# yanx27/PointASNL

Hardware: AMD Instinct MI355X
Metric: point-clouds/sec fwd (Bx1024 pts, ModelNet40 cls) (higher is better)
Workload: dtype f32; 1 GPU; configs[1]: ModelNet40 pointasnl_cls, 1024 pts, batch=64/GPU, seeded random weights; global_batch=64, parallelism=batch-shard x1, RCCL all-gather of logits, pipeline=prefetch, hip_graph=True, prefix_forked_at=start, prefix_levels=2, settle_replays=40, hip_hw_queues=4

## Files before the change

### include/pasnl.h

```cpp
#ifndef PASNL_H_
#define PASNL_H_

#include <stddef.h>
#include <stdint.h>

#ifdef __cplusplus
extern "C" {
#endif

#define PASNL_VERSION 100

enum {
  PASNL_OK = 0,
  PASNL_EINVAL = -1,
  PASNL_ENULL = -2,
  PASNL_EWORKSPACE = -3,
  PASNL_ELAUNCH = -4,
  PASNL_EUNSUPPORTED = -5
};

typedef void* pasnl_stream_t;

int pasnl_version(void);
const char* pasnl_strerror(int code);
// ... 92 lines not shown

int pasnl_sa_project(int b, int n, int c, int c1, const float* xyz, const float* feature, const float* w0, const float* b0,
                     float* proj, pasnl_stream_t stream);
int pasnl_sa_cell_pre(int b, int n, int c, int m, int k, int c1, int c2, const float* xyz, const float* feature,
                      const float* proj, const int* idx, const float* new_xyz, const float* w0, const float* w1, const float* b1,
                      const float* ww, const float* bw, float* out, float* skip_max, pasnl_stream_t stream);
int pasnl_sa_cell_pre_centre0(int b, int n, int c, int m, int k, int c1, int c2, const float* xyz, const float* feature,
                              const float* proj, const int* idx, const float* w0, const float* w1, const float* b1,
                              const float* ww, const float* bw, float* out, float* skip_max, float* new_xyz, float* new_feature,
                              pasnl_stream_t stream);

int pasnl_sa_cell_packed(int b, int n, int c, int npoint, int nsample, int c1, int c2, const float* xyz, const float* feature,
                         const int* idx, const float* new_xyz, const float* w0, const float* b0, const float* w1, const float* b1,
                         const float* ww, const float* bw, const float* w0_features_packed, const float* w1_packed, float* out,
                         float* skip_max, float* new_xyz_out, float* new_feature_out, pasnl_stream_t stream);

int pasnl_max_pool_rows(int b, int n, int c, const float* x, float* out, pasnl_stream_t stream);

int pasnl_max_pool_rows_strided(int b, int n, int c, const float* x, float* out, long out_stride, pasnl_stream_t stream);

size_t pasnl_mlp3_packed_weights_bytes(int k, int n);
int pasnl_mlp3_pack_weights(int k, int n, const float* w, float* packed, pasnl_stream_t stream);
size_t pasnl_mlp3_max_pool_workspace_bytes(int b, int n, int c3);
int pasnl_mlp3_max_pool(int b, int n, int k0, int c1, int c2, int c3, const float* x, const float* w0, const float* b0,
                        const float* w1, const float* b1, const float* w2, const float* b2, float* out, long out_stride,
                        void* workspace, size_t workspace_bytes, pasnl_stream_t stream);

int pasnl_cls_tail_group_all(int b, int n, int w, int cb, int c, const float* after, const float* skip_max, const float* att,
                             const float* ws_packed, const float* bs, const float* wb_packed, const float* bb,
                             const float* wagg_packed, const float* bagg, const float* new_xyz, int c1, int c2, int c3,
                             const float* w0, const float* b0, const float* w1, const float* b1, const float* w2, const float* b2,
                             float* out, float* pooled, long pooled_stride, void* workspace, size_t workspace_bytes,
                             pasnl_stream_t stream);

size_t pasnl_bf16x3_weights_bytes(int kdim, int n);
int pasnl_bf16x3_split_weights(int kdim, int n, const float* w, void* wsplit, pasnl_stream_t stream);
int pasnl_dense_bf16x3(int rows, int kdim, int n, int lda, const float* x, const void* wsplit, const float* bias, int relu,
                       float* out, pasnl_stream_t stream);


size_t pasnl_dense_rows_workspace_bytes(int rows, int kdim, int n);
int pasnl_dense_rows(int rows, int kdim, int n, const float* x, const float* w, const float* bias, int relu, float* out,
                     void* workspace, size_t workspace_bytes, pasnl_stream_t stream);

size_t pasnl_dense_splitk_workspace_bytes(int rows, int kdim, int n);
int pasnl_dense_splitk(int rows, int kdim, int n, int lda, const float* x, const float* w, const float* bias, int relu,
                       float* out, void* workspace, size_t workspace_bytes, pasnl_stream_t stream);

int pasnl_narrow_project2(long rows0, int kdim0, int n0, const float* x0, const float* w0, const float* bias0, float* out0,
                          long rows1, int kdim1, int n1, const float* x1, const float* w1, const float* bias1, float* out1,
                          pasnl_stream_t stream);

int pasnl_cls_nl_cell_input(int b, int p, int n, int c, int cz, int cb, const float* feature, const float* new_point,
                            const float* wkv, const float* bkv, const float* wq, const float* bq, float* out,
                            pasnl_stream_t stream);

size_t pasnl_cls_nl_cell_input_grad_workspace_bytes(int b, int p, int n, int c, int cz, int cb);
int pasnl_cls_nl_cell_input_grad(int b, int p, int n, int c, int cz, int cb, const float* feature, const float* new_point,
                                 const float* wkv, const float* bkv, const float* wq, const float* bq, const float* grad_out,
                                 float* grad_feature, float* grad_new_point, float* grad_wkv, float* grad_bkv, float* grad_wq,
                                 float* grad_bq, void* workspace, size_t workspace_bytes, pasnl_stream_t stream);

size_t pasnl_cls_nl_attention_grad_workspace_bytes(int b, int p, int n, int cb);
int pasnl_cls_nl_attention_grad(int b, int p, int n, int cb, const float* q, const float* kv, const float* out,
                                const float* grad_out, float* grad_q, float* grad_kv, void* workspace, size_t workspace_bytes,
                                pasnl_stream_t stream);
// ... 315 lines not shown
```

### pointasnl_amd/_hip.py

```python
import ctypes
import os

import torch

_HERE = os.path.dirname(os.path.abspath(__file__))
LIB_PATH = os.path.join(_HERE, "csrc", "libpasnl_hip.so")

SYMBOLS = [
    "pasnl_version", "pasnl_strerror", "pasnl_device_count",
    "pasnl_farthest_point_sample", "pasnl_farthest_point_sample_gather", "pasnl_gather_point", "pasnl_gather_point_grad", "pasnl_prob_sample",
    "pasnl_query_ball_point", "pasnl_sa_group", "pasnl_group_point", "pasnl_group_point_grad", "pasnl_select_top_k", "pasnl_knn_batch", "pasnl_knn_workspace_bytes", "pasnl_knn_batch_ws", "pasnl_knn_batch_ws_bg", "pasnl_knn_tree_workspace_bytes", "pasnl_knn_batch_tree", "pasnl_knn_batch_ref_workspace_bytes", "pasnl_knn_batch_ref", "pasnl_knn_distance_pick",
    "pasnl_three_nn", "pasnl_three_interpolate", "pasnl_three_interpolate_grad", "pasnl_three_weights", "pasnl_fp_interpolate_cat",
    "pasnl_nl_attention", "pasnl_nl_attention_workspace_bytes", "pasnl_nl_attention_ws", "pasnl_as_attention", "pasnl_as_reweight", "pasnl_sa_local_cell", "pasnl_sa_cell", "pasnl_sa_cell_centre0", "pasnl_sa_cell_packed", "pasnl_sa_project", "pasnl_sa_cell_pre", "pasnl_sa_cell_pre_centre0", "pasnl_sa_tail", "pasnl_sa_tail_cat", "pasnl_sa_tail_res", "pasnl_sa_tail_packed_weights_bytes", "pasnl_sa_tail_pack_weights", "pasnl_sa_tail_packed", "pasnl_decode_cell", "pasnl_decode_cell_tiled", "pasnl_decode_cell_tiled_v4", "pasnl_max_pool_rows", "pasnl_max_pool_rows_strided", "pasnl_mlp3_max_pool_workspace_bytes", "pasnl_mlp3_max_pool", "pasnl_mlp3_packed_weights_bytes", "pasnl_mlp3_pack_weights", "pasnl_dense_rows_workspace_bytes", "pasnl_dense_rows", "pasnl_dense_splitk_workspace_bytes", "pasnl_dense_splitk", "pasnl_bf16x3_weights_bytes", "pasnl_bf16x3_split_weights", "pasnl_dense_bf16x3", "pasnl_narrow_project2", "pasnl_take_neighbor0", "pasnl_as_gather", "pasnl_as_attention_qkv", "pasnl_as_attention_proj", "pasnl_as_cell_narrow", "pasnl_as_cell_wide", "pasnl_as_cell_wide_ld", "pasnl_as_reweight_x", "pasnl_grid_subsample_workspace_bytes", "pasnl_grid_subsample", "pasnl_knn_crop_workspace_bytes", "pasnl_knn_crop",
    "pasnl_scan_pick", "pasnl_knn_crop_indirect", "pasnl_crop_order_permute", "pasnl_scan_possibility_update", "pasnl_scan_scratch_init", "pasnl_scan_vote", "pasnl_scan_reproject_workspace_bytes", "pasnl_scan_reproject", "pasnl_scan_labels",
    "pasnl_scan_pick_given", "pasnl_scan_train_labels", "pasnl_scan_augment",
    "pasnl_scan_eval_confusion", "pasnl_scene_eval_vote", "pasnl_scene_eval_vote_confusion",
    "pasnl_scan_radius_workspace_bytes", "pasnl_scan_radius_members", "pasnl_scene_radius_members", "pasnl_scan_radius_gather", "pasnl_scene_radius_gather",
    "pasnl_scene_pick", "pasnl_knn_crop_scene", "pasnl_scene_pick_crop", "pasnl_scene_order_gather", "pasnl_scene_potential_update", "pasnl_scene_vote", "pasnl_scene_labels", "pasnl_confusion_matrix",
    "pasnl_window_noise", "pasnl_window_bounds", "pasnl_window_hist_bytes", "pasnl_window_count", "pasnl_window_fill", "pasnl_window_gather", "pasnl_window_vote", "pasnl_window_pool_labels",
    "pasnl_kwindow_hist_bytes", "pasnl_kwindow_count", "pasnl_kwindow_fill", "pasnl_kwindow_gather",
    "pasnl_modelnet_fps_cap", "pasnl_modelnet_fps", "pasnl_modelnet_normalize", "pasnl_modelnet_batch", "pasnl_modelnet_augment", "pasnl_modelnet_noise", "pasnl_cls_vote", "pasnl_cls_tally",
    "pasnl_cls_tail_group_all", "pasnl_cls_nl_cell_input", "pasnl_cls_nl_cell_input_grad_workspace_bytes", "pasnl_cls_nl_cell_input_grad", "pasnl_cls_nl_attention_grad_workspace_bytes", "pasnl_cls_nl_attention_grad",
    "pasnl_cls_as_attention_grad", "pasnl_cls_as_attention_qkv_grad", "pasnl_cls_as_reweight_grad", "pasnl_cls_as_reweight_x_grad", "pasnl_cls_as_gather_grad_workspace_bytes", "pasnl_cls_as_gather_grad",
    "pasnl_cls_sa_local_cell_grad_workspace_bytes", "pasnl_cls_sa_local_cell_grad", "pasnl_cls_sa_group_grad_workspace_bytes", "pasnl_cls_sa_group_grad",
    "pasnl_block_key_capacity", "pasnl_block_crop_stats", "pasnl_block_grid_count", "pasnl_block_fill", "pasnl_block_gather", "pasnl_block_normalize", "pasnl_block_score_workspace_bytes", "pasnl_block_score", "pasnl_block_train_batch", "pasnl_block_train_score",
    "pasnl_kblock_crop_stats", "pasnl_kblock_grid_count", "pasnl_kblock_fill", "pasnl_kblock_gather", "pasnl_kblock_rotate",
    "pasnl_grad_workspace_bytes", "pasnl_gather_point_grad_det", "pasnl_group_point_grad_det", "pasnl_three_interpolate_grad_det",
]


class PasnlError(RuntimeError):
    pass


class PasnlUnsupported(PasnlError):
    """PASNL_EUNSUPPORTED: a valid request outside what the fused kernel covers (include/pasnl.h documents the limits).
    The cells catch it and take their op-by-op path (still HIP kernels + vendor GEMMs, never a CPU path)."""


_lib = None


def lib():
    global _lib
    if _lib is None:
        if not os.path.exists(LIB_PATH):
            raise PasnlError(
                f"{LIB_PATH} is missing: build it with `python -c 'import __graft_entry__ as g; g.build()'` "
                "(or `make -C pointasnl_amd/csrc`).  pointasnl_amd has no CPU or eager fallback.")
        _lib = ctypes.CDLL(LIB_PATH)
        _lib.pasnl_strerror.restype = ctypes.c_char_p
        _lib.pasnl_grad_workspace_bytes.restype = ctypes.c_size_t
        _lib.pasnl_knn_workspace_bytes.restype = ctypes.c_size_t
        _lib.pasnl_knn_tree_workspace_bytes.restype = ctypes.c_size_t
        _lib.pasnl_knn_batch_ref_workspace_bytes.restype = ctypes.c_size_t
# ... 126 lines not shown
```

### pointasnl_amd/csrc/mlp_pool.hip

```cpp
#include "common.hpp"
#include "sa_tail.hpp"

namespace pasnl {

typedef float mp_f32x16 __attribute__((ext_vector_type(16)));

__device__ __forceinline__ int mp_kappa(int t, int h) { return (t & 3) + 8 * (t >> 2) + 4 * h; }

template <int WOUT, int NB, int RB>
__device__ __forceinline__ void mp_mm(const float* xrow, int rbstride, int NBT, const float* __restrict__ Wp, const int (&loff)[NB],
                                      mp_f32x16 (&acc)[RB][NB]) {
  constexpr int BT = 8;
  float xb[2][RB][BT];
  float4 wa[2][NB][2];
  auto load = [&](int set, int bt) {
    const float* wrow = Wp + (size_t)bt * (16 * WOUT);
#pragma unroll
    for (int i = 0; i < NB; ++i) {
      wa[set][i][0] = *reinterpret_cast<const float4*>(wrow + loff[i]);
      wa[set][i][1] = *reinterpret_cast<const float4*>(wrow + loff[i] + 4);
    }
#pragma unroll
    for (int u = 0; u < BT; ++u)
#pragma unroll
      for (int rb = 0; rb < RB; ++rb)
        xb[set][rb][u] = xrow[rb * rbstride + 2 * (bt * BT + u)];
  };
  load(0, 0);
  for (int bt = 0; bt < NBT; bt += 2) {
#pragma unroll
    for (int half = 0; half < 2; ++half) {
      const int b0 = bt + half;
      if (b0 < NBT) {
        load(half ^ 1, min(b0 + 1, NBT - 1));
        __builtin_amdgcn_sched_barrier(0);
#pragma unroll
        for (int u = 0; u < BT; ++u) {
          float wv[NB];
#pragma unroll
          for (int i = 0; i < NB; ++i) {
            const float4 q = wa[half][i][u >> 2];
            wv[i] = (u & 3) == 0 ? q.x : ((u & 3) == 1 ? q.y : ((u & 3) == 2 ? q.z : q.w));
          }
#pragma unroll
          for (int rb = 0; rb < RB; ++rb)
#pragma unroll
            for (int i = 0; i < NB; ++i)
              acc[rb][i] = __builtin_amdgcn_mfma_f32_32x32x2f32(xb[half][rb][u], wv[i], acc[rb][i], 0, 0, 0);
        }
        __builtin_amdgcn_sched_barrier(0);
      }
    }
  }
}

template <int WOUT, int RB>
__device__ __forceinline__ void mp_layer(const float* in, int pin, int K, const float* __restrict__ W, const float* __restrict__ bias,
                                         float* out, int pout, int wave, int ql, int h) {
  constexpr int NW = 8, BLOCKS = WOUT / 32, NB = BLOCKS >= NW ? BLOCKS / NW : 1;
  if constexpr (BLOCKS * RB == NW && RB > 1) {
    const int rb = wave / BLOCKS;
    mp_layer<WOUT, 1>(in + rb * 32 * pin, pin, K, W, bias, out + rb * 32 * pout, pout, wave % BLOCKS, ql, h);
    return;
  }
  if (wave >= BLOCKS) return;
  int loff[NB];
  mp_f32x16 acc[RB][NB];
#pragma unroll
  for (int i = 0; i < NB; ++i) {
    loff[i] = (h * WOUT + (wave + NW * i) * 32 + ql) * 8;
#pragma unroll
    for (int rb = 0; rb < RB; ++rb)
#pragma unroll
      for (int r = 0; r < 16; ++r) acc[rb][i][r] = 0.f;
  }
  mp_mm<WOUT, NB, RB>(in + ql * pin + h, 32 * pin, (K + 15) >> 4, W, loff, acc);
#pragma unroll
  for (int i = 0; i < NB; ++i) {
    const int ch = (wave + NW * i) * 32 + ql;
    const float bb = bias[ch];
#pragma unroll
    for (int rb = 0; rb < RB; ++rb)
#pragma unroll
      for (int r = 0; r < 16; ++r) out[(rb * 32 + mp_kappa(r, h)) * pout + ch] = fmaxf(acc[rb][i][r] + bb, 0.f);
  }
}

template <int C1, int C2, int C3, int RB>
__device__ __forceinline__ void mlp3_tile(float* A, int pa, float* Bf, int k0, const float* __restrict__ w0, const float* __restrict__ b0,
                                          const float* __restrict__ w1, const float* __restrict__ b1, const float* __restrict__ w2,
                                          const float* __restrict__ b2, float* __restrict__ po, int wave, int ql, int h) {
  constexpr int NW = 8, PB = C1 + 1;
  mp_layer<C1, RB>(A, pa, k0, w0, b0, Bf, PB, wave, ql, h);
  __syncthreads();
  mp_layer<C2, RB>(Bf, PB, C1, w1, b1, A, pa, wave, ql, h);
  __syncthreads();
  constexpr int NB = C3 / 32 / NW;
  int loff[NB];
  mp_f32x16 acc[RB][NB];
#pragma unroll
  for (int i = 0; i < NB; ++i) {
    loff[i] = (h * C3 + (wave + NW * i) * 32 + ql) * 8;
#pragma unroll
    for (int rb = 0; rb < RB; ++rb)
#pragma unroll
      for (int r = 0; r < 16; ++r) acc[rb][i][r] = 0.f;
  }
  mp_mm<C3, NB, RB>(A + ql * pa + h, 32 * pa, C2 >> 4, w2, loff, acc);
#pragma unroll
  for (int i = 0; i < NB; ++i) {
    float mx = acc[0][i][0];
#pragma unroll
    for (int rb = 0; rb < RB; ++rb)
#pragma unroll
      for (int r = 0; r < 16; ++r) mx = fmaxf(mx, acc[rb][i][r]);
    mx = fmaxf(mx, __shfl_xor(mx, 32));
    const int ch = (wave + NW * i) * 32 + ql;
// ... 94 lines not shown
    for (int i = 0; i < 16; ++i) v[i] = fmaxf(acc[i], 0.f);
#pragma unroll
    for (int i = 0; i < 16; ++i) acc[i] = bb[cbase + kappa(i, h)];
    acc = tail_product(TailW<true>{Wb, C, TG_CB, h, cbase + l32}, nt_, l32, acc);
#pragma unroll
    for (int i = 0; i < 16; ++i) v[i] += fmaxf(acc[i], 0.f);
#pragma unroll
    for (int i = 0; i < 16; ++i) {
      float* cell = vt + (cbase + kappa(i, h)) * 33 + l32;
      *cell = *cell + v[i];
    }
  }
  __syncthreads();
  {
    f32x16 o;
#pragma unroll
    for (int i = 0; i < 16; ++i) o[i] = bagg[cbase + kappa(i, h)];
    o = tail_product(TailW<true>{Wagg, C, C, h, cbase + l32}, vt, l32, o);
    float* xr = A + (rb * 32 + l32) * pa + 4 + cbase;
#pragma unroll
    for (int i = 0; i < 16; ++i) xr[kappa(i, h)] = fmaxf(o[i], 0.f);
  }
  __syncthreads();
#pragma unroll
  for (int i = 0; i < RPW; ++i) {
    const int r = wave * RPW + i, row = tile * TG_TR + r;
    if (row < n) {
      float* o = out + (cloud0 + row) * C;
      o[lane] = A[r * pa + 4 + lane];
      o[64 + lane] = A[r * pa + 4 + 64 + lane];
    }
  }
  mlp3_tile<TG_C, TG_C2, TG_C3, 2>(A, pa, Bf, TG_K0, w0, b0, w1, b1, w2, b2, partial + ((size_t)cloud * gridDim.x + tile) * TG_C3, wave, l32, h);
}

__global__ __launch_bounds__(256) void mlp3_pack_kernel(int K, int N, const float* __restrict__ W, float* __restrict__ P) {
  const long total = (long)((K + 15) >> 4) * 2 * N * 2;
  for (long e = (long)blockIdx.x * 256 + threadIdx.x; e < total; e += (long)gridDim.x * 256) {
    const int half = (int)(e & 1);
    const long lane = e >> 1;
    const int n = (int)(lane % N);
    const long bh = lane / N;
    const int h = (int)(bh & 1), bt = (int)(bh >> 1);
    float v[4];
#pragma unroll
    for (int j = 0; j < 4; ++j) {
      const int k = 16 * bt + 2 * (4 * half + j) + h;
      v[j] = k < K ? W[(size_t)k * N + n] : 0.f;
    }
    reinterpret_cast<float4*>(P)[e] = make_float4(v[0], v[1], v[2], v[3]);
  }
}

template <int C1, int C2, int C3, int RB>
static int mlp3_launch(int b, int n, int k0, const float* x, const float* w0, const float* b0, const float* w1, const float* b1,
                       const float* w2, const float* b2, float* partial, hipStream_t st) {
  const int k0p = (k0 + 15) & ~15;
  const int pa = (k0p > C2 ? k0p : C2) | 1;
  const size_t lds = ((size_t)32 * RB * pa + (size_t)32 * RB * (C1 + 1)) * sizeof(float);
  if (lds > LDS_MAX_BYTES) return PASNL_EUNSUPPORTED;
  if (launch(mlp3_pool_kernel<C1, C2, C3, RB>, dim3((n + 32 * RB - 1) / (32 * RB), b), dim3(512), lds, st, n, k0, x, w0, b0, w1, b1,
             w2, b2, partial) != PASNL_OK)
    return PASNL_ELAUNCH;
  return pasnl_launch_status();
}

// ... 36 lines not shown
  float* partial = static_cast<float*>(workspace);
  int rc;
  int tr;
  if (c1 == 128 && c2 == 256 && c3 == 512) { tr = 64; rc = mlp3_launch<128, 256, 512, 2>(b, n, k0, x, w0, b0, w1, b1, w2, b2, partial, st); }
  else if (c1 == 256 && c2 == 512 && c3 == 1024) { tr = 32; rc = mlp3_launch<256, 512, 1024, 1>(b, n, k0, x, w0, b0, w1, b1, w2, b2, partial, st); }
  else return PASNL_EUNSUPPORTED;
  if (rc != PASNL_OK) return rc;
  return pasnl_max_pool_rows_strided(b, (n + tr - 1) / tr, c3, partial, out, out_stride, stream);
}

extern "C" int pasnl_cls_tail_group_all(int b, int n, int w, int cb, int c, const float* after, const float* skip_max, const float* att,
                                        const float* ws_packed, const float* bs, const float* wb_packed, const float* bb,
                                        const float* wagg_packed, const float* bagg, const float* new_xyz, int c1, int c2, int c3,
                                        const float* w0, const float* b0, const float* w1, const float* b1, const float* w2,
                                        const float* b2, float* out, float* pooled, long pooled_stride, void* workspace,
                                        size_t workspace_bytes, pasnl_stream_t stream) {
  PASNL_REQUIRE(b >= 0 && n > 0 && w > 0 && cb > 0 && c > 0 && c1 > 0 && c2 > 0 && c3 > 0 && pooled_stride >= c3, PASNL_EINVAL);
  if (b == 0) return PASNL_OK;
  PASNL_REQUIRE(after && skip_max && att && ws_packed && bs && wb_packed && bb && wagg_packed && bagg && new_xyz, PASNL_ENULL);
  PASNL_REQUIRE(w0 && b0 && w1 && b1 && w2 && b2 && out && pooled && workspace, PASNL_ENULL);
  PASNL_REQUIRE(workspace_bytes >= pasnl_mlp3_max_pool_workspace_bytes(b, n, c3), PASNL_EWORKSPACE);
  PASNL_REQUIRE(w == TG_W && cb == TG_CB && c == TG_C && c1 == TG_C && c2 == TG_C2 && c3 == TG_C3, PASNL_EUNSUPPORTED);
  PASNL_REQUIRE(b <= 65535, PASNL_EUNSUPPORTED);
  PASNL_REQUIRE((reinterpret_cast<uintptr_t>(ws_packed) | reinterpret_cast<uintptr_t>(wb_packed) | reinterpret_cast<uintptr_t>(wagg_packed) |
                 reinterpret_cast<uintptr_t>(w0) | reinterpret_cast<uintptr_t>(w1) | reinterpret_cast<uintptr_t>(w2)) % 16 == 0,
                PASNL_EUNSUPPORTED);
  const int tiles = (n + TG_TR - 1) / TG_TR;
  if (launch(tail_group_all_kernel, dim3(tiles, b), dim3(512), TG_LDS_BYTES, pasnl_hip_stream(stream), n, after, skip_max, att, ws_packed,
             bs, wb_packed, bb, wagg_packed, bagg, new_xyz, w0, b0, w1, b1, w2, b2, out, static_cast<float*>(workspace)) != PASNL_OK)
    return PASNL_ELAUNCH;
  if (pasnl_launch_status() != PASNL_OK) return PASNL_ELAUNCH;
  return pasnl_max_pool_rows_strided(b, tiles, c3, static_cast<const float*>(workspace), pooled, pooled_stride, stream);
}
```

### pointasnl_amd/models/pointasnl_cls.py

```python
import torch

from pointasnl_amd.utils import tf_util, pointasnl_util
from pointasnl_amd.utils.pointnet_util import pointnet_sa_module
from pointasnl_amd.utils.pointasnl_util import PointASNLSetAbstraction, get_repulsion_loss, sa_search, Forked


def first_layer(num_point=None):
    return dict(npoint=512, nsample=32)


def get_model(point_cloud, is_training=False, use_normal=False, bn_decay=None, weight_decay=None, num_class=40,
              adaptive_sample=False, search=None, before_head=None, fork_at="head", lazy_fork=None):
    if lazy_fork is None:
        lazy_fork = not adaptive_sample
    batch_size = point_cloud.shape[0]
    end_points = {}
    if use_normal:
        l0_xyz = point_cloud[:, :, 0:3].contiguous()
        l0_points = point_cloud[:, :, 3:6].contiguous()
    else:
        l0_xyz = point_cloud
        l0_points = point_cloud
    end_points['l0_xyz'] = l0_xyz
    as_neighbor = [12, 12] if adaptive_sample else [0, 0]

    net = torch.empty((batch_size, 1024 + 512), dtype=torch.float32, device=point_cloud.device)
    fuse3_1 = not adaptive_sample or pointasnl_util.SA_TAIL_GROUP_ALL == "always"
    nl_input_space = not adaptive_sample or pointasnl_util.NL_INPUT_SPACE == "always"

    search2 = []
    if isinstance(search, dict):
        search2.append(search[2])
        search = search[1]
    l1_xyz, l1_points = PointASNLSetAbstraction(l0_xyz, l0_points, npoint=512, nsample=32, mlp=[64, 64, 128],
                                                is_training=is_training, bn_decay=bn_decay, weight_decay=weight_decay,
                                                scope='layer1', as_neighbor=as_neighbor[0], search=search, xyz_concat=True,
                                                nl_input_space=nl_input_space,
                                                group_all=dict(mlp=[128, 256, 512], scope='layer3_1', pooled_out=net[:, 1024:]) if fuse3_1 else None,
                                                after_sampling=None if search2 else lambda xyz1: search2.append(
                                                    Forked(lambda: sa_search(xyz1, None, 128, 64), lazy=lazy_fork)))
    end_points['l1_xyz'] = l1_xyz
    l2_xyz, l2_points = PointASNLSetAbstraction(l1_xyz, l1_points, npoint=128, nsample=64, mlp=[128, 128, 256],
                                                is_training=is_training, bn_decay=bn_decay, weight_decay=weight_decay,
                                                scope='layer2', as_neighbor=as_neighbor[1], search=search2[0], xyz_concat=True,
                                                after_cell=before_head if fork_at == "cell2" else None,
                                                before_after_conv=before_head if fork_at == "conv2" else None)
    end_points['l2_xyz'] = l1_xyz
    if before_head is not None and fork_at == "head":
        before_head()
    if getattr(l1_points, "group_all_pooled", None) is None:
        _, l3_points_res, _ = pointnet_sa_module(l1_xyz, l1_points, npoint=None, radius=None, nsample=None,
                                                 mlp=[128, 256, 512], mlp2=None, group_all=True, is_training=is_training,
                                                 bn_decay=bn_decay, scope='layer3_1', pooled_out=net[:, 1024:])
    _, l3_points, _ = pointnet_sa_module(l2_xyz, l2_points, npoint=None, radius=None, nsample=None,
                                         mlp=[256, 512, 1024], mlp2=None, group_all=True, is_training=is_training,
                                         bn_decay=bn_decay, scope='layer3_2', pooled_out=net[:, :1024])

    net = tf_util.fully_connected(net, 512, bn=True, is_training=is_training, scope='fc1', bn_decay=bn_decay)
    net = tf_util.dropout(net, keep_prob=0.4, is_training=is_training, scope='dp1')
    net = tf_util.fully_connected(net, 256, bn=True, is_training=is_training, scope='fc2', bn_decay=bn_decay)
    net = tf_util.dropout(net, keep_prob=0.4, is_training=is_training, scope='dp2')
    net = tf_util.fully_connected(net, num_class, activation_fn=None, scope='fc3')
    end_points['l1_points'] = l1_points
    end_points['l2_points'] = l2_points
    end_points['l2_xyz_true'] = l2_xyz
    return net, end_points


def get_loss(pred, label, end_points, uniform_weight=0, weights_decay=1e-4):
    regularization_loss = tf_util.regularization_loss(weights_decay)
    loss = torch.nn.functional.cross_entropy(pred, label.long(), reduction='none')
    classify_loss = loss.mean()
    if uniform_weight > 0:
        uniform_loss = get_repulsion_loss(end_points['l1_xyz'], nsample=20, radius=0.07)
    else:
        uniform_loss = classify_loss
    return classify_loss + uniform_weight * uniform_loss + regularization_loss
```

### pointasnl_amd/utils/pointasnl_util.py

```python

import ctypes

import torch

from pointasnl_amd import _hip
from pointasnl_amd import tf_sampling, tf_grouping, nearest_neighbors
from pointasnl_amd.tf_interpolate import three_nn, three_interpolate, three_weights, fp_interpolate_cat
from pointasnl_amd.utils import tf_util, pointnet_util

NL_KEY_PARTS = True
NL_VARIANT = 0


KNN_TIE_ORDER = "reference"


def knn_query(k, support_pts, query_pts, out=None, max_workgroups=None):
    return nearest_neighbors.knn_batch(support_pts, query_pts, k, omp=True, dtype=torch.int32, tie_order=KNN_TIE_ORDER, out=out,
                                       max_workgroups=max_workgroups)


def _gather_rows(points, idx):
    return tf_grouping.group_point(points, idx.unsqueeze(-1)).squeeze(2)

# ... 65 lines not shown
                    _hip.ptr(grad_new_xyz), _hip.ptr(ws), ctypes.c_size_t(nbytes))
        return grad_xyz, grad_feature, None, grad_new_xyz


def sa_group(xyz, feature, idx, new_xyz):
    if _needs_grad(xyz, feature, new_xyz):
        b, n, c = feature.shape
        _, p, k = idx.shape
        if _grad_entry_supported("pasnl_cls_sa_group_grad", b, n, c, p, k):
            return _SAGroup.apply(xyz, feature, idx, new_xyz)
        grouped_xyz = tf_grouping.group_point(xyz, idx)
        new_point = torch.cat([grouped_xyz - new_xyz.unsqueeze(2), grouped_xyz, tf_grouping.group_point(feature, idx)], dim=-1)
        return new_point, new_point.amax(dim=2)
    return _sa_group_forward(xyz, feature, idx, new_xyz)


def _sa_group_forward(xyz, feature, idx, new_xyz):
    b, n, c = feature.shape
    _, p, k = idx.shape
    xyz, feature, idx, new_xyz = xyz.contiguous(), feature.contiguous(), idx.contiguous(), new_xyz.contiguous()
    new_point = torch.empty((b, p, k, 6 + c), dtype=torch.float32, device=xyz.device)
    skip = torch.empty((b, p, 6 + c), dtype=torch.float32, device=xyz.device)
    _hip.launch("pasnl_sa_group", "sa_group", b, n, c, p, k, _hip.ptr(xyz), _hip.ptr(feature), _hip.ptr(idx),
                _hip.ptr(new_xyz), _hip.ptr(new_point), _hip.ptr(skip))
    return new_point, skip


SELF_KNN_RATIO = 2
SA_TAIL_MIN_ROWS = 2048
FP_HEAD_FUSED = True
SA_CELL_PACKED = True
SA_TAIL_PACKED = True
SA_TAIL_GROUP_ALL = True
SA_TAIL_FUSED = True
SA_CELL_GATHER = True
SA_CELL_SINGLE = True
SA_CELL_WIDE = True
LOCAL_CELL_FUSED = True


def _local_cell_supported(w, mlp, nsample):
    if not LOCAL_CELL_FUSED or nsample % 32:
        return False
    wide = (256, 512) if SA_CELL_WIDE else ()
    if len(mlp) == 3:
        return mlp[0] == mlp[1] and mlp[0] in (16, 32, 64, 128) + wide
    return len(mlp) == 2 and mlp[0] in (32, 64, 128) + wide


class _SALocalCell(torch.autograd.Function):

    @staticmethod
    def forward(ctx, new_point, w0, b0, w1, b1, ww, bw):
        args = tuple(t.contiguous() for t in (new_point, w0, b0, w1, b1, ww, bw))
        ctx.save_for_backward(*args)
        return _sa_local_cell_forward(*args)

    @staticmethod
    @torch.autograd.function.once_differentiable
    def backward(ctx, grad_out):
        x, w0, b0, w1, b1, ww, bw = ctx.saved_tensors
        b, p, k, w = x.shape
        c1, c2 = w0.shape[1], w1.shape[1]
        grad_out = grad_out.contiguous()
        grads = [torch.empty_like(t) if need else None for t, need in zip((x, w0, b0, w1, b1, ww, bw), ctx.needs_input_grad)]
        nbytes = int(_hip.lib().pasnl_cls_sa_local_cell_grad_workspace_bytes(b * p, w, c1, c2)) if any(ctx.needs_input_grad[1:]) else 0
# ... 807 lines not shown
def sa_search_split(xyz, npoint, nsample, knn_all, slot=0):
    fp = Forked(lambda: tf_sampling.farthest_point_sample_gather(npoint, xyz), slot=slot)

    def join():
        fps_idx, new_xyz = fp.get()
        k_all = _resolved(knn_all)
        idx = _gather_index_rows(k_all, fps_idx)
        if k_all.shape[2] != nsample:
            idx = idx[:, :, :nsample].contiguous()
        return new_xyz, None, idx
    return Deferred(join)


def _tail_packed(st, w):
    key = "@tailpk:%x" % w.data_ptr()
    if key not in st._folded:
        wc = w.contiguous()
        pk = torch.empty(int(_hip.lib().pasnl_sa_tail_packed_weights_bytes(wc.shape[0], wc.shape[1])) // 4, dtype=torch.float32,
                         device=w.device)
        _hip.launch("pasnl_sa_tail_pack_weights", "sa_tail_pack", int(wc.shape[0]), int(wc.shape[1]), _hip.ptr(wc), _hip.ptr(pk))
        st._folded[key] = (pk, w)
    return st._folded[key][0]


def PointASNLSetAbstraction(xyz, feature, npoint, nsample, mlp, is_training, bn_decay, weight_decay, scope, bn=True,
                            use_knn=True, radius=None, as_neighbor=8, NL=True, search=None, after_sampling=None,
                            xyz_concat=False, after_cell=None, before_after_conv=None, residual=None, group_all=None,
                            nl_input_space=True):
    ga_weights = None
    if (group_all is not None and SA_TAIL_GROUP_ALL and SA_TAIL_FUSED and SA_TAIL_PACKED and NL and residual is None and not is_training
            and mlp[-1] == 128 and tuple(group_all['mlp']) == (128, 256, 512)):
        with tf_util.variable_scope(group_all['scope']):
            ga_weights = pointnet_util.group_all_weights(group_all['mlp'], 3 + mlp[-1], 1, bn)
    with tf_util.variable_scope(scope):
        batch_size, num_points, num_channel = feature.shape
        new_xyz, _, idx = _resolved(search) if search is not None else sa_search(xyz, feature, npoint, nsample, use_knn, radius)
        new_feature = feature
        nl_channel = mlp[-1]
        st_path = tf_util.store().path("")
        diff = not is_training and torch.is_grad_enabled() and (
            xyz.requires_grad or feature.requires_grad
            or any(v.requires_grad for name, v in tf_util.store().vars.items() if name.startswith(st_path)))

        fused = _local_cell_supported(6 + num_channel, mlp, nsample)
        centre0 = False
        if num_points != npoint and as_neighbor == 0:
            xyz, feature, idx = xyz.contiguous(), feature.contiguous(), idx.contiguous()

            def take0():
                nx = torch.empty((batch_size, npoint, 3), dtype=torch.float32, device=xyz.device)
                nf = torch.empty((batch_size, npoint, 3 + num_channel), dtype=torch.float32, device=xyz.device)
                _hip.launch("pasnl_take_neighbor0", "take_neighbor0", batch_size, num_points, num_channel, npoint, nsample,
                            _hip.ptr(xyz), _hip.ptr(feature), _hip.ptr(idx), _hip.ptr(nx), _hip.ptr(nf))
                return nx, nf
            centre0 = (not diff and CENTRE0 and fused and SA_CELL_GATHER and npoint <= num_points
                       and (num_channel <= 128 or (SA_CELL_WIDE and mlp[0] in (256, 512) and nsample == 32)))
            if diff:
                idx0 = idx[:, :, 0].contiguous()
                new_xyz = _gather_rows(xyz, idx0)
                new_feature = torch.cat([new_xyz, _gather_rows(feature, idx0)], dim=-1)
            elif not centre0:
                new_xyz, new_feature = take0()
        elif num_points != npoint and AS_FUSED and as_neighbor <= 16:
            tf_util._require_inference(is_training)
            new_xyz, new_feature = adaptive_sampling_fused(xyz, feature, idx, as_neighbor, scope, bn, weight_decay)
        elif num_points != npoint:
# ... 60 lines not shown
                                   is_training=is_training, scope='after_conv', bn_decay=bn_decay, weight_decay=weight_decay)
            st = tf_util.store()
            w_in = skip_spatial.shape[-1]
            with tf_util.variable_scope('skip'):
                ws, bs = st.layer(w_in, c_out, bn, weight_decay)
            if NL:
                with tf_util.variable_scope(scope), tf_util.variable_scope('conv_back_project'):
                    wb, bb = st.layer(cb, c_out, bn, weight_decay)
            with tf_util.variable_scope('aggregation'):
                wagg, bagg = st.layer(c_out, c_out, bn, weight_decay)
            rows = batch_size * npoint
            after, skip_spatial = after.contiguous(), skip_spatial.contiguous()
            att = att.contiguous() if NL else None
            out = torch.empty((batch_size, npoint, c_out), dtype=torch.float32, device=xyz.device)
            args = (rows, int(w_in), int(cb if NL else 0), int(c_out), _hip.ptr(after), _hip.ptr(skip_spatial),
                    _hip.ptr(att), _hip.ptr(ws), _hip.ptr(bs), _hip.ptr(wb if NL else None),
                    _hip.ptr(bb if NL else None), _hip.ptr(wagg), _hip.ptr(bagg), _hip.ptr(out))
            try:
                if SA_TAIL_PACKED:
                    pk = [_tail_packed(st, m) if m is not None else None for m in (ws, wb if NL else None, wagg)]
                    cat = None
                    if ga_weights is not None and (int(w_in), int(cb)) == (9, 32) and new_xyz.shape[1] == npoint:
                        new_xyz = new_xyz.contiguous()
                        gmlp = group_all['mlp']
                        pooled = pointnet_util.group_all_pooled(group_all.get('pooled_out'), batch_size, gmlp[-1], xyz.device)
                        wsb = pointnet_util.group_all_workspace(batch_size, npoint, gmlp[-1], xyz.device)
                        _hip.launch("pasnl_cls_tail_group_all", "sa_tail_group_all", batch_size, npoint, int(w_in), int(cb), int(c_out),
                                    *args[4:7], _hip.ptr(pk[0]), args[8], _hip.ptr(pk[1]), args[10], _hip.ptr(pk[2]), args[12],
                                    _hip.ptr(new_xyz), gmlp[0], gmlp[1], gmlp[2], *[_hip.ptr(t) for t in ga_weights], args[13],
                                    _hip.ptr(pooled), ctypes.c_long(pooled.stride(0) if batch_size > 1 else gmlp[-1]),
                                    _hip.ptr(wsb), ctypes.c_size_t(wsb.numel()))
                        out.group_all_pooled = pooled
                        return new_xyz, out
                    if xyz_concat and XYZ_CONCAT:
                        new_xyz = new_xyz.contiguous()
                        cat = torch.empty((batch_size, npoint, 4 + c_out), dtype=torch.float32, device=xyz.device)
                    res_c = residual.contiguous() if residual is not None else None
                    _hip.launch("pasnl_sa_tail_packed", "sa_tail", *args[:7], _hip.ptr(pk[0]), args[8], _hip.ptr(pk[1]), args[10],
                                _hip.ptr(pk[2]), args[12], _hip.ptr(res_c), _hip.ptr(new_xyz if cat is not None else None),
                                _hip.ptr(cat), args[13])
                    residual = None
                    if cat is not None:
                        out.xyz_concat = (new_xyz, cat)
                elif residual is not None:
                    residual = residual.contiguous()
                    _hip.launch("pasnl_sa_tail_res", "sa_tail", *args[:-1], _hip.ptr(residual), args[-1])
                    residual = None
                elif xyz_concat and XYZ_CONCAT:
                    new_xyz = new_xyz.contiguous()
                    cat = torch.empty((batch_size, npoint, 4 + c_out), dtype=torch.float32, device=xyz.device)
                    _hip.launch("pasnl_sa_tail_cat", "sa_tail", *args, _hip.ptr(new_xyz), _hip.ptr(cat))
                    out.xyz_concat = (new_xyz, cat)
                else:
                    _hip.launch("pasnl_sa_tail", "sa_tail", *args)
            except _hip.PasnlUnsupported:
                tail = after.reshape(rows, c_out) + torch.relu_(torch.addmm(bs, skip_spatial.reshape(rows, w_in), ws))
                if NL:
                    tail = tail + torch.relu_(torch.addmm(bb, att.reshape(rows, cb), wb))
                out = torch.relu_(torch.addmm(bagg, tail, wagg)).reshape(batch_size, npoint, c_out)
            return new_xyz, (out if residual is None else out + residual)

        if NL:
            new_nonlocal_point = PointNonLocalCell(feature, new_feature.unsqueeze(1),
                                                   [max(32, num_channel // 2), nl_channel], is_training, bn_decay,
                                                   weight_decay, scope, bn, input_space=nl_input_space)

# ... 117 lines not shown
```

### pointasnl_amd/utils/pointnet_util.py

```python
import ctypes

import torch

from pointasnl_amd.tf_sampling import farthest_point_sample, farthest_point_sample_gather, gather_point
from pointasnl_amd.tf_grouping import query_ball_point, group_point, knn_point
from pointasnl_amd.tf_interpolate import three_nn, three_interpolate, three_weights, fp_interpolate_cat
from pointasnl_amd.utils import tf_util
from pointasnl_amd import _hip


def sample_and_group(npoint, radius, nsample, xyz, points, knn=False, use_xyz=True):
    _, new_xyz = farthest_point_sample_gather(npoint, xyz)
    if knn:
        _, idx = knn_point(nsample, xyz, new_xyz)
    else:
        idx, pts_cnt = query_ball_point(radius, nsample, xyz, new_xyz)
    grouped_xyz = group_point(xyz, idx)
    grouped_xyz = grouped_xyz - new_xyz.unsqueeze(2)
    if points is not None:
        grouped_points = group_point(points, idx)
        new_points = torch.cat([grouped_xyz, grouped_points], dim=-1) if use_xyz else grouped_points
    else:
        new_points = grouped_xyz
    return new_xyz, new_points, idx, grouped_xyz
# ... 32 lines not shown
                if key not in st._folded:
                    st._folded[key] = (torch.cat([w.new_zeros((pad, w.shape[1])), w], dim=0).contiguous(), bb)
                w, bb = st._folded[key]
            key = st.path("") + "@mlp3:%x" % w.data_ptr()
            if key not in st._folded:
                wc = w.contiguous()
                pk = torch.empty(int(_hip.lib().pasnl_mlp3_packed_weights_bytes(wc.shape[0], wc.shape[1])) // 4, dtype=torch.float32,
                                 device=w.device)
                _hip.launch("pasnl_mlp3_pack_weights", "mlp3_pack", int(wc.shape[0]), int(wc.shape[1]), _hip.ptr(wc), _hip.ptr(pk))
                st._folded[key] = (pk, w)
            w = st._folded[key][0]
        ws += [w, bb]
        cin = c
    return ws


def group_all_pooled(pooled_out, b, c3, device):
    if pooled_out is None:
        return torch.empty((b, c3), dtype=torch.float32, device=device)
    if tuple(pooled_out.shape) != (b, c3) or pooled_out.stride(1) != 1 or pooled_out.dtype != torch.float32:
        raise ValueError("group_all_mlp_max: pooled_out must be a (B, C) float32 view with unit column stride")
    return pooled_out


def group_all_workspace(b, n, c3, device):
    nbytes = int(_hip.lib().pasnl_mlp3_max_pool_workspace_bytes(b, n, c3))
    key = (device.index, torch.cuda.current_stream().cuda_stream, c3)
    bufs = _GROUP_ALL_WS.setdefault(key, [])
    if not bufs or bufs[-1].numel() < nbytes:
        bufs.append(torch.empty(max(nbytes, 256), dtype=torch.uint8, device=device))
    return bufs[-1]


def group_all_mlp_max(new_points, mlp, bn, pooled_out=None):
    b, one, n, kp = new_points.shape
    if one != 1 or len(mlp) != 3:
        raise _hip.PasnlUnsupported("group_all_mlp_max: one group per cloud, three convolutions")
    pad = getattr(new_points, "input_pad", 0)
    ws = group_all_weights(mlp, kp - pad, pad, bn)
    x = new_points.reshape(b, n, kp)
    if not x.is_contiguous():
        x = x.contiguous()
    c3 = mlp[-1]
    out2d = group_all_pooled(pooled_out, b, c3, x.device)
    wsb = group_all_workspace(b, n, c3, x.device)
    _hip.launch("pasnl_mlp3_max_pool", "mlp3_max_pool", b, n, kp, mlp[0], mlp[1], mlp[2], _hip.ptr(x), *[_hip.ptr(t) for t in ws],
                _hip.ptr(out2d), ctypes.c_long(out2d.stride(0) if b > 1 else c3), _hip.ptr(wsb), ctypes.c_size_t(wsb.numel()))
    return out2d.unflatten(0, (b, 1)).unsqueeze(2)


def sample_and_group_all(xyz, points, use_xyz=True):
    batch_size, nsample = xyz.shape[0], xyz.shape[1]
    key = (batch_size, nsample, str(xyz.device))
    if key not in _GROUP_ALL_CONST:
        new_xyz = torch.zeros((batch_size, 1, 3), dtype=torch.float32, device=xyz.device)
        idx = torch.arange(nsample, dtype=torch.int32, device=xyz.device).reshape(1, 1, nsample).repeat(batch_size, 1, 1)
        _GROUP_ALL_CONST[key] = (new_xyz, idx)
    new_xyz, idx = _GROUP_ALL_CONST[key]
    grouped_xyz = xyz.reshape(batch_size, 1, nsample, 3)
    pre = getattr(points, "xyz_concat", None) if (points is not None and use_xyz) else None
    if pre is not None and pre[0] is xyz:
        new_points = pre[1].unsqueeze(1)
        new_points.input_pad = 1
    elif points is not None:
        new_points = torch.cat([xyz, points], dim=2) if use_xyz else points
        new_points = new_points.unsqueeze(1)
# ... 55 lines not shown
```

### pointasnl_amd/utils/tf_util.py

```python
import contextlib
import hashlib
import math

import numpy as np
import torch

from pointasnl_amd import _hip

BN_EPS = 1e-3
FUSE_RELU_EPILOGUE = True
WEIGHTS_TRANSPOSED_MIN_K = 2048


class VariableStore:

    def __init__(self, seed=0, device="cuda", randomize_bn=False):
        self.seed = int(seed)
        self.device = device
        self.randomize_bn = randomize_bn
        self.vars = {}
        self.decays = {}
        self._folded = {}
        self._scope = []

    @contextlib.contextmanager
    def scope(self, name):
        self._scope.append(name)
        try:
            yield
        finally:
            self._scope.pop()

    def path(self, name):
        return "/".join(self._scope + [name])

    def _rng(self, full):
        h = hashlib.sha256(f"{self.seed}:{full}".encode()).digest()
        return np.random.Generator(np.random.PCG64(int.from_bytes(h[:8], "little")))

    def load(self, variables, strict=True):
        for name in getattr(variables, "files", None) or variables.keys():
            leaf = name.split(":")[0].split("/")[-1]
            if leaf not in ("weights", "biases", "beta", "gamma", "moving_mean", "moving_variance"):
                continue
            a = np.asarray(variables[name], dtype=np.float32)
            if leaf == "weights" and a.ndim > 2:
                a = a.reshape(-1, a.shape[-1])
            self.vars[name.split(":")[0]] = torch.tensor(a, dtype=torch.float32, device=self.device)
        self.strict = bool(strict)
        self._folded.clear()
        return self

    def assign(self, full_name, value):
        self.vars[full_name] = torch.as_tensor(value, dtype=torch.float32).to(self.device).contiguous()
        self._folded.clear()

    strict = False

    def get(self, name, shape, kind):
        full = self.path(name)
        if full in self.vars and tuple(self.vars[full].shape) != tuple(shape):
            raise ValueError(f"variable {full}: stored shape {tuple(self.vars[full].shape)} but the layer needs {tuple(shape)}")
        if full not in self.vars and self.strict:
            raise KeyError(f"variable {full} {tuple(shape)} is not in the loaded checkpoint (VariableStore.load(strict=True))")
# ... 271 lines not shown
```

Baseline: 59340 point-clouds/s.

## Fuse layer2 SA tail with first two layer3_2 group-all MLP layers

```diff
diff --git a/include/pasnl.h b/include/pasnl.h
--- a/include/pasnl.h
+++ b/include/pasnl.h
@@ -148,6 +148,12 @@
                              const float* w0, const float* b0, const float* w1, const float* b1, const float* w2, const float* b2,
                              float* out, float* pooled, long pooled_stride, void* workspace, size_t workspace_bytes,
                              pasnl_stream_t stream);
+
+int pasnl_cls_tail_mlp2(int b, int n, int w, int cb, int c, const float* after, const float* skip_max, const float* att,
+                        const float* ws_packed, const float* bs, const float* wb_packed, const float* bb,
+                        const float* wagg_packed, const float* bagg, const float* new_xyz, int c1, int c2, const float* w0,
+                        const float* b0, const float* w1, const float* b1, float* out, float* h2, size_t h2_bytes,
+                        pasnl_stream_t stream);
 
 size_t pasnl_bf16x3_weights_bytes(int kdim, int n);
 int pasnl_bf16x3_split_weights(int kdim, int n, const float* w, void* wsplit, pasnl_stream_t stream);
diff --git a/pointasnl_amd/_hip.py b/pointasnl_amd/_hip.py
--- a/pointasnl_amd/_hip.py
+++ b/pointasnl_amd/_hip.py
@@ -20,7 +20,7 @@
     "pasnl_window_noise", "pasnl_window_bounds", "pasnl_window_hist_bytes", "pasnl_window_count", "pasnl_window_fill", "pasnl_window_gather", "pasnl_window_vote", "pasnl_window_pool_labels",
     "pasnl_kwindow_hist_bytes", "pasnl_kwindow_count", "pasnl_kwindow_fill", "pasnl_kwindow_gather",
     "pasnl_modelnet_fps_cap", "pasnl_modelnet_fps", "pasnl_modelnet_normalize", "pasnl_modelnet_batch", "pasnl_modelnet_augment", "pasnl_modelnet_noise", "pasnl_cls_vote", "pasnl_cls_tally",
-    "pasnl_cls_tail_group_all", "pasnl_cls_nl_cell_input", "pasnl_cls_nl_cell_input_grad_workspace_bytes", "pasnl_cls_nl_cell_input_grad", "pasnl_cls_nl_attention_grad_workspace_bytes", "pasnl_cls_nl_attention_grad",
+    "pasnl_cls_tail_group_all", "pasnl_cls_tail_mlp2", "pasnl_cls_nl_cell_input", "pasnl_cls_nl_cell_input_grad_workspace_bytes", "pasnl_cls_nl_cell_input_grad", "pasnl_cls_nl_attention_grad_workspace_bytes", "pasnl_cls_nl_attention_grad",
     "pasnl_cls_as_attention_grad", "pasnl_cls_as_attention_qkv_grad", "pasnl_cls_as_reweight_grad", "pasnl_cls_as_reweight_x_grad", "pasnl_cls_as_gather_grad_workspace_bytes", "pasnl_cls_as_gather_grad",
     "pasnl_cls_sa_local_cell_grad_workspace_bytes", "pasnl_cls_sa_local_cell_grad", "pasnl_cls_sa_group_grad_workspace_bytes", "pasnl_cls_sa_group_grad",
     "pasnl_block_key_capacity", "pasnl_block_crop_stats", "pasnl_block_grid_count", "pasnl_block_fill", "pasnl_block_gather", "pasnl_block_normalize", "pasnl_block_score_workspace_bytes", "pasnl_block_score", "pasnl_block_train_batch", "pasnl_block_train_score",
diff --git a/pointasnl_amd/csrc/mlp_pool.hip b/pointasnl_amd/csrc/mlp_pool.hip
--- a/pointasnl_amd/csrc/mlp_pool.hip
+++ b/pointasnl_amd/csrc/mlp_pool.hip
@@ -56,7 +56,7 @@
 
 template <int WOUT, int RB>
 __device__ __forceinline__ void mp_layer(const float* in, int pin, int K, const float* __restrict__ W, const float* __restrict__ bias,
-                                         float* out, int pout, int wave, int ql, int h) {
+                                         float* out, int pout, int wave, int ql, int h, int rows = 32 * RB) {
   constexpr int NW = 8, BLOCKS = WOUT / 32, NB = BLOCKS >= NW ? BLOCKS / NW : 1;
   if constexpr (BLOCKS * RB == NW && RB > 1) {
     const int rb = wave / BLOCKS;
@@ -82,7 +82,9 @@
 #pragma unroll
     for (int rb = 0; rb < RB; ++rb)
 #pragma unroll
-      for (int r = 0; r < 16; ++r) out[(rb * 32 + mp_kappa(r, h)) * pout + ch] = fmaxf(acc[rb][i][r] + bb, 0.f);
+      for (int r = 0; r < 16; ++r)
+        if (rb * 32 + mp_kappa(r, h) < rows)
+          out[(rb * 32 + mp_kappa(r, h)) * pout + ch] = fmaxf(acc[rb][i][r] + bb, 0.f);
   }
 }
 
@@ -243,6 +245,110 @@
     }
   }
   mlp3_tile<TG_C, TG_C2, TG_C3, 2>(A, pa, Bf, TG_K0, w0, b0, w1, b1, w2, b2, partial + ((size_t)cloud * gridDim.x + tile) * TG_C3, wave, l32, h);
+}
+
+constexpr int T2_C = 256, T2_W = 134, T2_CB = 64, T2_K0 = T2_C + 4, T2_C1 = 256, T2_C2 = 512, T2_TR = 32;
+constexpr int T2_K0P = (T2_K0 + 15) & ~15;
+constexpr int T2_PA = T2_K0P | 1;
+constexpr int T2_WP = (T2_W + 2 * TAIL_KS - 1) & ~(2 * TAIL_KS - 1);
+constexpr int T2_TAIL_FLOATS = (T2_C + T2_WP + T2_CB) * 33;
+constexpr int T2_H1_FLOATS = T2_TR * (T2_C1 + 1);
+constexpr size_t T2_LDS_BYTES = ((size_t)T2_TR * T2_PA + (T2_TAIL_FLOATS > T2_H1_FLOATS ? T2_TAIL_FLOATS : T2_H1_FLOATS)) * sizeof(float);
+static_assert(T2_LDS_BYTES <= LDS_MAX_BYTES, "X rows + the tail's tiles fit one workgroup's LDS");
+static_assert(T2_C == 8 * 32 && T2_C1 == 8 * 32 && T2_C2 % 256 == 0 && T2_C % 64 == 0 && T2_CB == 64 && T2_WP <= 192 && T2_K0P - T2_K0 <= 60,
+              "one channel block per wave; the staging's segment counts");
+
+__global__ __launch_bounds__(512) void tail_mlp2_kernel(int n, const float* __restrict__ after, const float* __restrict__ S,
+                                                        const float* __restrict__ N, const float* __restrict__ Ws,
+                                                        const float* __restrict__ bs, const float* __restrict__ Wb,
+                                                        const float* __restrict__ bb, const float* __restrict__ Wagg,
+                                                        const float* __restrict__ bagg, const float* __restrict__ xyz3,
+                                                        const float* __restrict__ w0, const float* __restrict__ b0,
+                                                        const float* __restrict__ w1, const float* __restrict__ b1,
+                                                        float* __restrict__ out, float* __restrict__ h2) {
+  constexpr int C = T2_C, pa = T2_PA, RPW = T2_TR / 8, SA = C / 64, SS = (T2_WP + 63) / 64;
+  extern __shared__ __attribute__((aligned(16))) char smem[];
+  float* A = reinterpret_cast<float*>(smem);
+  float* Bf = A + T2_TR * pa;
+  float* vt = Bf;
+  float* st = vt + C * 33;
+  float* nt_ = st + T2_WP * 33;
+  const int tid = threadIdx.x, lane = tid & 63, wave = tid >> 6, h = lane >> 5, l32 = lane & 31;
+  const int tile = blockIdx.x, cloud = blockIdx.y;
+  const long cloud0 = (long)cloud * n;
+  {
+    float va[SA][RPW], vs[SS][RPW], vn[RPW], cx[RPW];
+#pragma unroll
+    for (int i = 0; i < RPW; ++i) {
+      const long row = cloud0 + min(tile * T2_TR + wave * RPW + i, n - 1);
+#pragma unroll
+      for (int s = 0; s < SA; ++s) va[s][i] = after[row * C + s * 64 + lane];
+#pragma unroll
+      for (int s = 0; s < SS; ++s) vs[s][i] = S[row * T2_W + min(s * 64 + lane, T2_W - 1)];
+      vn[i] = N[row * T2_CB + lane];
+      cx[i] = xyz3[row * 3 + max(min(lane, 3) - 1, 0)];
+    }
+    __builtin_amdgcn_sched_barrier(0);
+#pragma unroll
+    for (int i = 0; i < RPW; ++i) {
+      const int r = wave * RPW + i;
+#pragma unroll
+      for (int s = 0; s < SA; ++s) vt[(s * 64 + lane) * 33 + r] = va[s][i];
+#pragma unroll
+      for (int s = 0; s < SS; ++s) {
+        const int c = s * 64 + lane;
+        if (c < T2_WP) st[c * 33 + r] = c < T2_W ? vs[s][i] : 0.f;
+      }
+      nt_[lane * 33 + r] = vn[i];
+      float* xr = A + r * pa;
+      if (lane < 4) xr[lane] = lane ? cx[i] : 0.f;
+      else if (lane < 4 + T2_K0P - T2_K0) xr[T2_K0 + lane - 4] = 0.f;
+    }
+  }
+  __syncthreads();
+  const int cbase = wave * 32;
+  {
+    f32x16 acc;
+#pragma unroll
+    for (int i = 0; i < 16; ++i) acc[i] = bs[cbase + kappa(i, h)];
+    acc = tail_product(TailW<true>{Ws, C, T2_W, h, cbase + l32}, st, l32, acc);
+    f32x16 v;
+#pragma unroll
+    for (int i = 0; i < 16; ++i) v[i] = fmaxf(acc[i], 0.f);
+#pragma unroll
+    for (int i = 0; i < 16; ++i) acc[i] = bb[cbase + kappa(i, h)];
+    acc = tail_product(TailW<true>{Wb, C, T2_CB, h, cbase + l32}, nt_, l32, acc);
+#pragma unroll
+    for (int i = 0; i < 16; ++i) v[i] += fmaxf(acc[i], 0.f);
+#pragma unroll
+    for (int i = 0; i < 16; ++i) {
+      float* cell = vt + (cbase + kappa(i, h)) * 33 + l32;
+      *cell = *cell + v[i];
+    }
+  }
+  __syncthreads();
+  {
+    f32x16 o;
+#pragma unroll
+    for (int i = 0; i < 16; ++i) o[i] = bagg[cbase + kappa(i, h)];
+    o = tail_product(TailW<true>{Wagg, C, C, h, cbase + l32}, vt, l32, o);
+    float* xr = A + l32 * pa + 4 + cbase;
+#pragma unroll
+    for (int i = 0; i < 16; ++i) xr[kappa(i, h)] = fmaxf(o[i], 0.f);
+  }
+  __syncthreads();
+#pragma unroll
+  for (int i = 0; i < RPW; ++i) {
+    const int r = wave * RPW + i, row = tile * T2_TR + r;
+    if (row < n) {
+      float* o = out + (cloud0 + row) * C;
+#pragma unroll
+      for (int s = 0; s < SA; ++s) o[s * 64 + lane] = A[r * pa + 4 + s * 64 + lane];
+    }
+  }
+  mp_layer<T2_C1, 1>(A, pa, T2_K0, w0, b0, Bf, T2_C1 + 1, wave, l32, h);
+  __syncthreads();
+  mp_layer<T2_C2, 1>(Bf, T2_C1 + 1, T2_C1, w1, b1, h2 + (cloud0 + (long)tile * T2_TR) * T2_C2, T2_C2, wave, l32, h, n - tile * T2_TR);
 }
 
 __global__ __launch_bounds__(256) void mlp3_pack_kernel(int K, int N, const float* __restrict__ W, float* __restrict__ P) {
@@ -345,3 +451,24 @@
   if (pasnl_launch_status() != PASNL_OK) return PASNL_ELAUNCH;
   return pasnl_max_pool_rows_strided(b, tiles, c3, static_cast<const float*>(workspace), pooled, pooled_stride, stream);
 }
+
+extern "C" int pasnl_cls_tail_mlp2(int b, int n, int w, int cb, int c, const float* after, const float* skip_max, const float* att,
+                                   const float* ws_packed, const float* bs, const float* wb_packed, const float* bb,
+                                   const float* wagg_packed, const float* bagg, const float* new_xyz, int c1, int c2, const float* w0,
+                                   const float* b0, const float* w1, const float* b1, float* out, float* h2, size_t h2_bytes,
+                                   pasnl_stream_t stream) {
+  PASNL_REQUIRE(b >= 0 && n > 0 && w > 0 && cb > 0 && c > 0 && c1 > 0 && c2 > 0, PASNL_EINVAL);
+  if (b == 0) return PASNL_OK;
+  PASNL_REQUIRE(after && skip_max && att && ws_packed && bs && wb_packed && bb && wagg_packed && bagg && new_xyz, PASNL_ENULL);
+  PASNL_REQUIRE(w0 && b0 && w1 && b1 && out && h2, PASNL_ENULL);
+  PASNL_REQUIRE(w == T2_W && cb == T2_CB && c == T2_C && c1 == T2_C1 && c2 == T2_C2, PASNL_EUNSUPPORTED);
+  PASNL_REQUIRE(h2_bytes >= (size_t)b * n * c2 * sizeof(float), PASNL_EWORKSPACE);
+  PASNL_REQUIRE(b <= 65535, PASNL_EUNSUPPORTED);
+  PASNL_REQUIRE((reinterpret_cast<uintptr_t>(ws_packed) | reinterpret_cast<uintptr_t>(wb_packed) | reinterpret_cast<uintptr_t>(wagg_packed) |
+                 reinterpret_cast<uintptr_t>(w0) | reinterpret_cast<uintptr_t>(w1)) % 16 == 0,
+                PASNL_EUNSUPPORTED);
+  if (launch(tail_mlp2_kernel, dim3((n + T2_TR - 1) / T2_TR, b), dim3(512), T2_LDS_BYTES, pasnl_hip_stream(stream), n, after, skip_max, att,
+             ws_packed, bs, wb_packed, bb, wagg_packed, bagg, new_xyz, w0, b0, w1, b1, out, h2) != PASNL_OK)
+    return PASNL_ELAUNCH;
+  return pasnl_launch_status();
+}
diff --git a/pointasnl_amd/models/pointasnl_cls.py b/pointasnl_amd/models/pointasnl_cls.py
--- a/pointasnl_amd/models/pointasnl_cls.py
+++ b/pointasnl_amd/models/pointasnl_cls.py
@@ -27,6 +27,7 @@
     net = torch.empty((batch_size, 1024 + 512), dtype=torch.float32, device=point_cloud.device)
     fuse3_1 = not adaptive_sample or pointasnl_util.SA_TAIL_GROUP_ALL == "always"
     nl_input_space = not adaptive_sample or pointasnl_util.NL_INPUT_SPACE == "always"
+    fuse3_2 = not adaptive_sample or pointasnl_util.SA_TAIL_MLP2 == "always"
 
     search2 = []
     if isinstance(search, dict):
@@ -43,6 +44,7 @@
     l2_xyz, l2_points = PointASNLSetAbstraction(l1_xyz, l1_points, npoint=128, nsample=64, mlp=[128, 128, 256],
                                                 is_training=is_training, bn_decay=bn_decay, weight_decay=weight_decay,
                                                 scope='layer2', as_neighbor=as_neighbor[1], search=search2[0], xyz_concat=True,
+                                                group_all=dict(mlp=[256, 512, 1024], scope='layer3_2', pooled_out=net[:, :1024]) if fuse3_2 else None,
                                                 after_cell=before_head if fork_at == "cell2" else None,
                                                 before_after_conv=before_head if fork_at == "conv2" else None)
     end_points['l2_xyz'] = l1_xyz
@@ -52,9 +54,10 @@
         _, l3_points_res, _ = pointnet_sa_module(l1_xyz, l1_points, npoint=None, radius=None, nsample=None,
                                                  mlp=[128, 256, 512], mlp2=None, group_all=True, is_training=is_training,
                                                  bn_decay=bn_decay, scope='layer3_1', pooled_out=net[:, 1024:])
-    _, l3_points, _ = pointnet_sa_module(l2_xyz, l2_points, npoint=None, radius=None, nsample=None,
-                                         mlp=[256, 512, 1024], mlp2=None, group_all=True, is_training=is_training,
-                                         bn_decay=bn_decay, scope='layer3_2', pooled_out=net[:, :1024])
+    if getattr(l2_points, "group_all_pooled", None) is None:
+        _, l3_points, _ = pointnet_sa_module(l2_xyz, l2_points, npoint=None, radius=None, nsample=None,
+                                             mlp=[256, 512, 1024], mlp2=None, group_all=True, is_training=is_training,
+                                             bn_decay=bn_decay, scope='layer3_2', pooled_out=net[:, :1024])
 
     net = tf_util.fully_connected(net, 512, bn=True, is_training=is_training, scope='fc1', bn_decay=bn_decay)
     net = tf_util.dropout(net, keep_prob=0.4, is_training=is_training, scope='dp1')
diff --git a/pointasnl_amd/utils/pointasnl_util.py b/pointasnl_amd/utils/pointasnl_util.py
--- a/pointasnl_amd/utils/pointasnl_util.py
+++ b/pointasnl_amd/utils/pointasnl_util.py
@@ -121,6 +121,7 @@
 SA_CELL_PACKED = True
 SA_TAIL_PACKED = True
 SA_TAIL_GROUP_ALL = True
+SA_TAIL_MLP2 = True
 SA_TAIL_FUSED = True
 SA_CELL_GATHER = True
 SA_CELL_SINGLE = True
@@ -994,6 +995,12 @@
             and mlp[-1] == 128 and tuple(group_all['mlp']) == (128, 256, 512)):
         with tf_util.variable_scope(group_all['scope']):
             ga_weights = pointnet_util.group_all_weights(group_all['mlp'], 3 + mlp[-1], 1, bn)
+    mlp2_weights = mlp2_scope = None
+    if (group_all is not None and SA_TAIL_MLP2 and SA_TAIL_FUSED and SA_TAIL_PACKED and NL and residual is None and not is_training
+            and mlp[-1] == 256 and tuple(group_all['mlp']) == (256, 512, 1024)):
+        with tf_util.variable_scope(group_all['scope']):
+            mlp2_weights = pointnet_util.group_all_weights(group_all['mlp'][:2], 3 + mlp[-1], 1, bn)
+            mlp2_scope = list(tf_util.store()._scope)
     with tf_util.variable_scope(scope):
         batch_size, num_points, num_channel = feature.shape
         new_xyz, _, idx = _resolved(search) if search is not None else sa_search(xyz, feature, npoint, nsample, use_knn, radius)
@@ -1120,6 +1127,21 @@
                                     _hip.ptr(wsb), ctypes.c_size_t(wsb.numel()))
                         out.group_all_pooled = pooled
                         return new_xyz, out
+                    if mlp2_weights is not None and (int(w_in), int(cb)) == (134, 64) and new_xyz.shape[1] == npoint:
+                        new_xyz = new_xyz.contiguous()
+                        gmlp = group_all['mlp']
+                        h2 = torch.empty((batch_size, 1, npoint, gmlp[1]), dtype=torch.float32, device=xyz.device)
+                        try:
+                            _hip.launch("pasnl_cls_tail_mlp2", "sa_tail_mlp2", batch_size, npoint, int(w_in), int(cb), int(c_out),
+                                        *args[4:7], _hip.ptr(pk[0]), args[8], _hip.ptr(pk[1]), args[10], _hip.ptr(pk[2]), args[12],
+                                        _hip.ptr(new_xyz), gmlp[0], gmlp[1], *[_hip.ptr(t) for t in mlp2_weights], args[13],
+                                        _hip.ptr(h2), ctypes.c_size_t(h2.numel() * 4))
+                        except _hip.PasnlUnsupported:
+                            h2 = None
+                        if h2 is not None:
+                            with tf_util.store().scope_at(mlp2_scope):
+                                out.group_all_pooled = pointnet_util.group_all_last(h2, gmlp[2], bn, group_all.get('pooled_out'))
+                            return new_xyz, out
                     if xyz_concat and XYZ_CONCAT:
                         new_xyz = new_xyz.contiguous()
                         cat = torch.empty((batch_size, npoint, 4 + c_out), dtype=torch.float32, device=xyz.device)
diff --git a/pointasnl_amd/utils/pointnet_util.py b/pointasnl_amd/utils/pointnet_util.py
--- a/pointasnl_amd/utils/pointnet_util.py
+++ b/pointasnl_amd/utils/pointnet_util.py
@@ -88,6 +88,13 @@
     return bufs[-1]
 
 
+def group_all_last(h2, c3, bn, pooled_out=None):
+    x = tf_util.conv2d(h2, c3, [1, 1], padding='VALID', stride=[1, 1], bn=bn, is_training=False, scope='conv2')
+    out2d = group_all_pooled(pooled_out, h2.shape[0], c3, h2.device)
+    max_pool_points(x, out=out2d)
+    return out2d
+
+
 def group_all_mlp_max(new_points, mlp, bn, pooled_out=None):
     b, one, n, kp = new_points.shape
     if one != 1 or len(mlp) != 3:
diff --git a/pointasnl_amd/utils/tf_util.py b/pointasnl_amd/utils/tf_util.py
--- a/pointasnl_amd/utils/tf_util.py
+++ b/pointasnl_amd/utils/tf_util.py
@@ -30,6 +30,14 @@
             yield
         finally:
             self._scope.pop()
+
+    @contextlib.contextmanager
+    def scope_at(self, names):
+        saved, self._scope = self._scope, list(names)
+        try:
+            yield
+        finally:
+            self._scope = saved
 
     def path(self, name):
         return "/".join(self._scope + [name])
```

Measured after the change: 60350 point-clouds/s, median of 6. 1.7% higher.
